# yanqinJiang/Animate3D

Measured on AMD Instinct MI355X. Metric: UNet denoise-steps/sec, 4view×16frame×512² MV-VDM @1/2/4/8 GPU, higher is better.
Workload: dtype bf16; 1 GPU; BASELINE config 2: 4 views x 16 frames x 512^2 px (64x64 latent), CFG-doubled batch V=8 videos, one MVUNetMotionModel.forward per step, SD1.5 MV-VDM UNet 1.53 B params, seeded synthetic weights; parallelism=single GPU

## Files before the change

### animate3d_amd/csrc/gemm_common.h

```cpp
#pragma once
#include "common.h"

struct GemmParams {
  const uint16_t* X; int64_t ldx;
  const uint16_t* W; int64_t ldw;
  const float* bias;
  const uint16_t* rowbias; int64_t rb_div;
  const uint16_t* R; int64_t ldr;
  uint16_t* Y; int64_t ldy;
  int64_t M, N, K;
  float alpha, beta;
  int vec16;
  int out_f32;
  int B, H, Wd, Cin, Ho, Wo, stride, up, He, We;
  int64_t tiles_n, tiles_m;
  int ksplit, nk_item;
  float* ws; int64_t ws_bytes;
  const uint16_t* X2; int64_t ldx2; int64_t K1;
};

constexpr int EPI_LINEAR = 0, EPI_GEGLU = 1;

static inline int a3d_gemm_kernel_of(int flags) { return flags & A3D_GEMM_KERNEL_MASK; }
static inline int a3d_gemm_reserved_cus_of(int flags) { return flags & A3D_GEMM_RESERVED_CUS_MASK; }
// ... 321 lines not shown
      const float4 a1 = *reinterpret_cast<const float4*>(stg + row * SROW + 8 * cc + 4);
      float v[8] = {a0.x, a0.y, a0.z, a0.w, a1.x, a1.y, a1.z, a1.w};
#pragma unroll
      for (int e = 0; e < 8; ++e) v[e] += bv[e];
#pragma unroll
      for (int e = 0; e < 4; ++e) { v[2 * e] += lo16(tb[e]); v[2 * e + 1] += hi16(tb[e]); }
#pragma unroll
      for (int e = 0; e < 8; ++e) v[e] = epi_scale(v[e], p.alpha);
      const u32x4_t tr = rres[pi & 1][j];
#pragma unroll
      for (int e = 0; e < 4; ++e) { v[2 * e] = epi_axpy(v[2 * e], p.beta, lo16(tr[e])); v[2 * e + 1] = epi_axpy(v[2 * e + 1], p.beta, hi16(tr[e])); }
      u32x4_t o;
#pragma unroll
      for (int e = 0; e < 4; ++e) o[e] = pack16(v[2 * e], v[2 * e + 1]);
      *reinterpret_cast<u32x4_t*>(p.Y + m * p.ldy + n) = o;
    }
    wave_lds_fence();
  }
}


__attribute__((visibility("hidden"))) int A3D_FN(a3d_launch_gemm_pp)(int conv, int epi, int nb, hipStream_t stream, const GemmParams& p, int cus);
__attribute__((visibility("hidden"))) int A3D_FN(a3d_launch_gemm_ring)(int nb, hipStream_t stream, const GemmParams& p, int cus);
```

### animate3d_amd/csrc/gemm_conv.hip

```cpp
#include "gemm_common.h"

namespace {

constexpr int BM = 128, BN = 128;
template <int BKT> struct TileCfg {
  static constexpr int LROW = BKT + 8;
  static constexpr int TILE_ELEMS = 128 * LROW;
  static constexpr int STAGE_BYTES = 2 * 2 * TILE_ELEMS * 2;
  static constexpr int EPI_BYTES = 4 * 32 * 68 * 4;
  static constexpr int SMEM_BYTES = STAGE_BYTES > EPI_BYTES ? STAGE_BYTES : EPI_BYTES;
  static constexpr int CPR = BKT / 8;
  static constexpr int RPT = 256 / CPR;
  static constexpr int NPASS = 128 / RPT;
};



template <int CONV, int EPI, int BKT, bool RES>
__global__ __launch_bounds__(256, (BKT == 64 ? 2 : 3)) void gemm_kernel(const GemmParams p) {
  using TC = TileCfg<BKT>;
  constexpr int LROW = TC::LROW, TILE_ELEMS = TC::TILE_ELEMS, NPASS = TC::NPASS, RPT = TC::RPT, BK = BKT;
  extern __shared__ __attribute__((aligned(16))) uint16_t smem[];
  const int tid = threadIdx.x;
  const int lane = tid & 63, wid = tid >> 6;
// ... 491 lines not shown
                                void* Y, int64_t ldy, int64_t M, int64_t N, int64_t K, float alpha, float beta, int flags,
                                void* ws, int64_t ws_bytes, int64_t* ws_needed) {
  return gemm_entry(stream, X, ldx, W, ldw, bias, rowbias, rb_div, R, ldr, Y, ldy, M, N, K, alpha, beta, flags, ws, ws_bytes, ws_needed);
}

extern "C" int A3D_FN(a3d_gemm2)(a3d_stream_t stream, const void* X, int64_t ldx, const void* X2, int64_t ldx2, int64_t K1,
                              const void* W, int64_t ldw, const float* bias, void* Y, int64_t ldy, int64_t M, int64_t N, int64_t K, int flags) {
  GemmParams p = dense_params(X, ldx, W, ldw, bias, nullptr, 1, nullptr, 0, Y, ldy, M, N, K, 1.f, 0.f);
  p.X2 = (const uint16_t*)X2; p.ldx2 = ldx2; p.K1 = K1;
  if (!dense_args_ok(p, 16, 8, 8) || !X2 || K1 <= 0 || K1 >= K || K1 % 64 != 0 || ldx2 % 8 != 0 || !a3d_aligned(16, X2)) return A3D_EINVAL;
  if (!gemm_flags_ok(flags)) return A3D_EINVAL;
  if (ldx2 % 64 != 0 || (uint64_t)ldx2 * 16u >= (1ull << 31)) return A3D_EUNSUPPORTED;
  const int rc = try_launch_persist<0, EPI_LINEAR>((hipStream_t)stream, p, flags);
  return rc == NOT_ELIGIBLE ? A3D_EUNSUPPORTED : rc;
}

extern "C" int A3D_FN(a3d_gemm_f32out)(a3d_stream_t stream, const void* X, int64_t ldx, const void* W, int64_t ldw,
                                    const float* bias, float* Y, int64_t ldy, int64_t M, int64_t N, int64_t K, float alpha) {
  GemmParams p = dense_params(X, ldx, W, ldw, bias, nullptr, 1, nullptr, 0, Y, ldy, M, N, K, alpha, 0.f, true);
  if (!dense_args_ok(p, 16, 8, 4)) return A3D_EINVAL;
  return launch<0>((hipStream_t)stream, p, 0);
}

static int conv_entry(a3d_stream_t stream, const void* X, const void* Wp, const float* bias,
                      const void* rowbias, int64_t rb_div, const void* R, void* Y,
                      int B, int H, int W, int Cin, int Cout, int stride, int up2x, int flags,
                      void* ws, int64_t ws_bytes, int64_t* ws_needed) {
  if (!X || !Wp || !Y || B <= 0 || H <= 0 || W <= 0) return A3D_EINVAL;
  if (Cin % 64 != 0 || Cout % 4 != 0 || (stride != 1 && stride != 2)) return A3D_EINVAL;
  if (up2x < 0 || up2x > 7 || (up2x > 1 && !(up2x & 1)) || (up2x && stride != 1)) return A3D_EINVAL;
  if (!a3d_aligned(16, X, Wp) || !a3d_aligned(16, bias) || !a3d_aligned(8, Y)) return A3D_EINVAL;
  if (rowbias && rb_div <= 0) return A3D_EINVAL;
  const int He = up2x ? 2 * H - ((up2x >> 1) & 1) : H, We = up2x ? 2 * W - ((up2x >> 2) & 1) : W;
  if (He <= 0 || We <= 0) return A3D_EINVAL;
  GemmParams p{};
  p.X = (const uint16_t*)X; p.ldx = Cin; p.W = (const uint16_t*)Wp; p.ldw = (int64_t)9 * Cin;
  p.bias = bias; p.rowbias = (const uint16_t*)rowbias; p.rb_div = rowbias ? rb_div : 1;
  p.R = (const uint16_t*)R; p.ldr = Cout; p.Y = (uint16_t*)Y; p.ldy = Cout;
  p.B = B; p.H = H; p.Wd = W; p.Cin = Cin; p.stride = stride; p.up = up2x ? 1 : 0; p.He = He; p.We = We;
  p.Ho = (He + 2 - 3) / stride + 1; p.Wo = (We + 2 - 3) / stride + 1;
  p.M = (int64_t)B * p.Ho * p.Wo; p.N = Cout; p.K = (int64_t)9 * Cin;
  p.alpha = 1.f; p.beta = 1.f;
  p.vec16 = (Cout % 8 == 0) && a3d_aligned(16, Y, R, rowbias);
  if (ws_needed) { *ws_needed = up2x ? splitk_ws_bytes<2>(p, flags) : splitk_ws_bytes<1>(p, flags); return 0; }
  attach_workspace(p, ws, ws_bytes);
  return up2x ? launch<2>((hipStream_t)stream, p, flags) : launch<1>((hipStream_t)stream, p, flags);
}

extern "C" int A3D_FN(a3d_conv3x3)(a3d_stream_t stream, const void* X, const void* Wp, const float* bias,
                                const void* rowbias, int64_t rb_div, const void* R, void* Y,
                                int B, int H, int W, int Cin, int Cout, int stride, int up2x, int flags) {
  return conv_entry(stream, X, Wp, bias, rowbias, rb_div, R, Y, B, H, W, Cin, Cout, stride, up2x, flags, nullptr, 0, nullptr);
}

extern "C" int A3D_FN(a3d_conv3x3_ws)(a3d_stream_t stream, const void* X, const void* Wp, const float* bias,
                                   const void* rowbias, int64_t rb_div, const void* R, void* Y,
                                   int B, int H, int W, int Cin, int Cout, int stride, int up2x, int flags,
                                   void* ws, int64_t ws_bytes, int64_t* ws_needed) {
  return conv_entry(stream, X, Wp, bias, rowbias, rb_div, R, Y, B, H, W, Cin, Cout, stride, up2x, flags, ws, ws_bytes, ws_needed);
}

extern "C" int A3D_FN(a3d_gemm_geglu)(a3d_stream_t stream, const void* X, int64_t ldx, const void* W, int64_t ldw,
                                   const float* bias, void* Y, int64_t ldy, int64_t M, int64_t N2, int64_t K, int flags) {
  GemmParams p = dense_params(X, ldx, W, ldw, bias, nullptr, 1, nullptr, 0, Y, ldy, M, N2, K, 1.f, 0.f);
  if (!dense_args_ok(p, 16, 64, 8)) return A3D_EINVAL;
  return launch<0, EPI_GEGLU>((hipStream_t)stream, p, flags);
}
```

### animate3d_amd/csrc/temporal_attn.hip

```cpp
#include "common.h"


namespace {

constexpr int SLAB = 320;
constexpr int SL = 40;
constexpr int NSL = SLAB / SL;

struct TAParams {
  const uint16_t* Q; const uint16_t* K; const uint16_t* V; int64_t ld;
  int64_t ldq;
  uint16_t* O; int64_t ldo;
  int videos, frames; int64_t L; int heads; float scale_log2;
  int64_t npix;
  int q_f0, q_frames, kv_fpr; int64_t kv_rs;
};

typedef short s16x4_t __attribute__((ext_vector_type(4)));
typedef _Float16 f16x4_t __attribute__((ext_vector_type(4)));
A3D_DEV f32x4_t mfma16k16(const u32x2_t& a, const u32x2_t& b, const f32x4_t& c) {
#ifdef A3D_STORAGE_F16
  return __builtin_amdgcn_mfma_f32_16x16x16f16(__builtin_bit_cast(f16x4_t, a), __builtin_bit_cast(f16x4_t, b), c, 0, 0, 0);
#else
  return __builtin_amdgcn_mfma_f32_16x16x16bf16_1k(__builtin_bit_cast(s16x4_t, a), __builtin_bit_cast(s16x4_t, b), c, 0, 0, 0);
#endif
}

template <int FP, int D>
__global__ __launch_bounds__(NSL * FP) void temporal_attn_mfma_kernel(const TAParams p) {
  constexpr int ROWB = SLAB + 8;
  constexpr int FB = FP / 16;
  constexpr int KS = (D + 15) / 16;
  constexpr int NH = SLAB / D;
  constexpr int NT = NSL * FP, NW = NT / 64;
  extern __shared__ __attribute__((aligned(16))) uint16_t smem[];
  const int F = p.frames;
  const int tid = threadIdx.x, lane = tid & 63, wid = tid >> 6;
  const int64_t pix = blockIdx.x < p.npix ? (int64_t)blockIdx.x : p.npix - 1;
  const int c0 = blockIdx.y * SLAB;
  const int64_t v = pix / p.L, l = pix % p.L;
  constexpr int chunks = SLAB / 8;

  auto src_of = [&](int it) -> const uint16_t* {
    const int ch = it % chunks;
    const int f = (it / chunks) % F;
    const int ten = it / (chunks * F);
    if (ten == 0) {
      int fq = f - p.q_f0;
      if (fq < 0 || fq >= p.q_frames) fq = 0;
      return p.Q + ((v * p.q_frames + fq) * p.L + l) * p.ldq + c0 + ch * 8;
    }
    const int64_t row = (int64_t)(f / p.kv_fpr) * p.kv_rs + (v * p.kv_fpr + f % p.kv_fpr) * p.L + l;
    return (ten == 1 ? p.K : p.V) + row * p.ld + c0 + ch * 8;
  };
  auto dst_of = [&](int it) -> uint16_t* {
    const int ch = it % chunks;
    const int f = (it / chunks) % F;
    const int ten = it / (chunks * F);
    return smem + ((size_t)ten * F + f) * ROWB + ch * 8;
  };
  const int items = 3 * F * chunks;
  if (F == FP) {
    constexpr int ITEMS = 3 * FP * chunks, NIT = (ITEMS + NT - 1) / NT;
    u32x4_t stg[NIT];
#pragma unroll
    for (int k = 0; k < NIT; ++k) {
      const int it = tid + k * NT;
      if (ITEMS % NT == 0 || it < ITEMS) stg[k] = *reinterpret_cast<const u32x4_t*>(src_of(it));
    }
#pragma unroll
    for (int k = 0; k < NIT; ++k) {
      const int it = tid + k * NT;
      if (ITEMS % NT == 0 || it < ITEMS) *reinterpret_cast<u32x4_t*>(dst_of(it)) = stg[k];
    }
  } else {
    for (int it = tid; it < items; it += NT) *reinterpret_cast<u32x4_t*>(dst_of(it)) = *reinterpret_cast<const u32x4_t*>(src_of(it));
  }
  __syncthreads();

  const int i16 = lane & 15, k4 = lane >> 4;
  uint16_t* const Qs = smem;
  const uint16_t* const Ks = smem + (size_t)F * ROWB;
  const uint16_t* const Vs = smem + (size_t)2 * F * ROWB;
  for (int h = wid; h < NH; h += NW) {
    const int hc = h * D;
    f32x4_t sT[FB][FB];
    u32x2_t qfr[FB][KS];
#pragma unroll
    for (int ib = 0; ib < FB; ++ib) {
      const int fi = 16 * ib + i16 < F ? 16 * ib + i16 : F - 1;
#pragma unroll
      for (int ks = 0; ks < KS; ++ks) {
        u32x2_t w = *reinterpret_cast<const u32x2_t*>(Qs + (size_t)fi * ROWB + hc + 16 * ks + 4 * k4);
        if (16 * ks + 4 * k4 >= D) w = u32x2_t{0u, 0u};
        qfr[ib][ks] = w;
      }
    }
#pragma unroll
    for (int jb = 0; jb < FB; ++jb) {
      const int fj = 16 * jb + i16 < F ? 16 * jb + i16 : F - 1;
      u32x2_t kfr[KS];
#pragma unroll
      for (int ks = 0; ks < KS; ++ks) {
        kfr[ks] = *reinterpret_cast<const u32x2_t*>(Ks + (size_t)fj * ROWB + hc + 16 * ks + 4 * k4);
        if (16 * ks + 4 * k4 >= D) kfr[ks] = u32x2_t{0u, 0u};
      }
#pragma unroll
      for (int ib = 0; ib < FB; ++ib) {
        f32x4_t acc = {0.f, 0.f, 0.f, 0.f};
#pragma unroll
        for (int ks = 0; ks < KS; ++ks) acc = mfma16k16(kfr[ks], qfr[ib][ks], acc);
        sT[jb][ib] = acc;
      }
    }
    u32x2_t pfr[FB][FB];
    float inv[FB];
#pragma unroll
    for (int ib = 0; ib < FB; ++ib) {
      float mx = -INFINITY;
#pragma unroll
      for (int jb = 0; jb < FB; ++jb)
#pragma unroll
        for (int r = 0; r < 4; ++r) {
          const bool ok = 16 * jb + 4 * k4 + r < F;
          sT[jb][ib][r] = ok ? sT[jb][ib][r] * p.scale_log2 : -INFINITY;
          mx = fmaxf(mx, sT[jb][ib][r]);
        }
      mx = fmaxf(mx, __shfl_xor(mx, 16));
      mx = fmaxf(mx, __shfl_xor(mx, 32));
      float sum = 0.f;
#pragma unroll
      for (int jb = 0; jb < FB; ++jb) {
        float e[4];
#pragma unroll
        for (int r = 0; r < 4; ++r) { e[r] = __builtin_amdgcn_exp2f(sT[jb][ib][r] - mx); sum += e[r]; }
        pfr[jb][ib] = u32x2_t{pack16(e[0], e[1]), pack16(e[2], e[3])};
      }
      sum += __shfl_xor(sum, 16);
      sum += __shfl_xor(sum, 32);
      inv[ib] = 1.f / sum;
    }
#pragma unroll
    for (int db = 0; db < KS; ++db) {
      u32x2_t vfr[FB];
#pragma unroll
      for (int jb = 0; jb < FB; ++jb) {
        const int fj = 16 * jb + 4 * k4 + (i16 >> 2) < F ? 16 * jb + 4 * k4 + (i16 >> 2) : F - 1;
        vfr[jb] = lds_tr16_b64(Vs + (size_t)fj * ROWB + hc + 16 * db + 4 * (i16 & 3));
      }
#pragma unroll
      for (int ib = 0; ib < FB; ++ib) {
        f32x4_t o = {0.f, 0.f, 0.f, 0.f};
#pragma unroll
        for (int jb = 0; jb < FB; ++jb) o = mfma16k16(vfr[jb], pfr[jb][ib], o);
        const int fi = 16 * ib + i16;
        if (16 * db + 4 * k4 < D && fi < F) {
          const u32x2_t w = {pack16(o[0] * inv[ib], o[1] * inv[ib]), pack16(o[2] * inv[ib], o[3] * inv[ib])};
          *reinterpret_cast<u32x2_t*>(Qs + (size_t)fi * ROWB + hc + 16 * db + 4 * k4) = w;
        }
      }
    }
  }
  __syncthreads();
  if ((int64_t)blockIdx.x < p.npix) {
    for (int it = tid; it < p.q_frames * chunks; it += NT) {
      const int ch = it % chunks, fq = it / chunks;
      const u32x4_t w = *reinterpret_cast<const u32x4_t*>(Qs + (size_t)(p.q_f0 + fq) * ROWB + ch * 8);
      *reinterpret_cast<u32x4_t*>(p.O + ((v * p.q_frames + fq) * p.L + l) * p.ldo + c0 + ch * 8) = w;
    }
  }
}

template <int FP, int D>
int launch_mfma(hipStream_t s, const TAParams& p, int C) {
  if (p.npix > 0x7fffffffLL) return A3D_EINVAL;
  const size_t lds = (size_t)3 * p.frames * (SLAB + 8) * sizeof(uint16_t);
  static uint64_t attr_done = 0;
  if (int rc = a3d_once_per_device(attr_done, [] {
        return (int)hipFuncSetAttribute(reinterpret_cast<const void*>(&temporal_attn_mfma_kernel<FP, D>),
                                        hipFuncAttributeMaxDynamicSharedMemorySize, 3 * FP * (SLAB + 8) * 2); })) return rc;
  temporal_attn_mfma_kernel<FP, D><<<dim3((unsigned)p.npix, (unsigned)(C / SLAB)), dim3(NSL * FP), lds, s>>>(p);
  return a3d_launch_status();
}

template <int DP>
int launch_dp(hipStream_t s, const TAParams& p, int C) {
  if (p.frames <= 16) return launch_mfma<16, 40 * DP>(s, p, C);
  return launch_mfma<32, 40 * DP>(s, p, C);
}

}

static int temporal_attn_launch(a3d_stream_t stream, const void* Q, int64_t ldq, const void* K, const void* V, int64_t ldqkv, void* O, int64_t ldo,
                                int videos, int frames, int64_t L, int heads, int head_dim, float scale,
                                int q_f0, int q_frames, int kv_fpr, int64_t kv_rs) {
  if (!Q || !K || !V || !O || videos <= 0 || frames <= 0 || frames > 32 || L <= 0 || heads <= 0) return A3D_EINVAL;
  if (q_f0 < 0 || q_frames <= 0 || q_f0 + q_frames > frames || kv_fpr <= 0 || frames % kv_fpr != 0 || kv_rs < 0) return A3D_EINVAL;
  if (ldqkv % 8 || ldo % 8 || ldq % 8) return A3D_EINVAL;
  if ((reinterpret_cast<uintptr_t>(Q) | reinterpret_cast<uintptr_t>(K) | reinterpret_cast<uintptr_t>(V) |
       reinterpret_cast<uintptr_t>(O)) & 15u) return A3D_EINVAL;
  const int C = heads * head_dim;
  if (C % SLAB != 0) return A3D_EUNSUPPORTED;
  TAParams p{};
  p.Q = (const uint16_t*)Q; p.K = (const uint16_t*)K; p.V = (const uint16_t*)V; p.ld = ldqkv; p.ldq = ldq;
  p.O = (uint16_t*)O; p.ldo = ldo; p.videos = videos; p.frames = frames; p.L = L; p.heads = heads;
  p.scale_log2 = scale * 1.4426950408889634f;
  p.npix = (int64_t)videos * L;
  p.q_f0 = q_f0; p.q_frames = q_frames; p.kv_fpr = kv_fpr; p.kv_rs = kv_rs;
  hipStream_t s = (hipStream_t)stream;
  switch (head_dim) {
    case 40: return launch_dp<1>(s, p, C);
    case 80: return launch_dp<2>(s, p, C);
    case 160: return launch_dp<4>(s, p, C);
    default: return A3D_EUNSUPPORTED;
// ... 17 lines not shown
```

### animate3d_amd/hip_ops.py

```python
from __future__ import annotations

import ctypes
import os
from dataclasses import dataclass
from typing import Optional

import torch

_LIB_PATH = os.path.join(os.path.dirname(os.path.abspath(__file__)), "lib", "libanimate3d_hip.so")
_lib = None

c_i64, c_int, c_f32, c_f64, c_vp = ctypes.c_int64, ctypes.c_int, ctypes.c_float, ctypes.c_double, ctypes.c_void_p


class _RowMapC(ctypes.Structure):
    _fields_ = [("gdiv", c_i64), ("ga", c_i64), ("gb", c_i64), ("seg_len", c_i64), ("seg_stride", c_i64), ("ld", c_i64)]


class StageAdamEntry(ctypes.Structure):
    _fields_ = [("p", c_vp), ("g", c_vp), ("m", c_vp), ("v", c_vp), ("step", c_vp), ("n", c_i64), ("lr", c_f64)]


STAGE_ADAM_MAX_TENSORS = 32
STAGE_ADAM_BEGIN, STAGE_ADAM_CHECK, STAGE_ADAM_UPDATE = 1, 2, 4
# ... 14 lines not shown
def rowmap_rows(m: RowMap, groups: int, step: int, length: int, device="cpu") -> torch.Tensor:
    g = torch.arange(0, groups, step, device=device).view(-1, 1)
    s = torch.arange(length, device=device).view(1, -1)
    return ((g // m.gdiv) * m.ga + (g % m.gdiv) * m.gb + (s // m.seg_len) * m.seg_stride + s % m.seg_len).reshape(-1)


def rowmap_covers(m: RowMap, groups: int, step: int, length: int, rows: int, device="cpu") -> bool:
    if (groups + step - 1) // step * length != rows:
        return False
    idx = rowmap_rows(m, groups, step, length, device)
    return bool(int(idx.min()) >= 0 and int(idx.max()) < rows and torch.unique(idx).numel() == rows)


_SIGNATURES = {
    "a3d_version": (ctypes.c_char_p, []),
    "a3d_gemm_bf16": (c_int, [c_vp, c_vp, c_i64, c_vp, c_i64, c_vp, c_vp, c_i64, c_vp, c_i64, c_vp, c_i64, c_i64, c_i64, c_i64, c_f32, c_f32, c_int]),
    "a3d_gemm_ws_bf16": (c_int, [c_vp, c_vp, c_i64, c_vp, c_i64, c_vp, c_vp, c_i64, c_vp, c_i64, c_vp, c_i64, c_i64, c_i64, c_i64, c_f32, c_f32, c_int,
                                 c_vp, c_i64, ctypes.POINTER(c_i64)]),
    "a3d_gemm2_bf16": (c_int, [c_vp, c_vp, c_i64, c_vp, c_i64, c_i64, c_vp, c_i64, c_vp, c_vp, c_i64, c_i64, c_i64, c_i64, c_int]),
    "a3d_gemm_geglu_bf16": (c_int, [c_vp, c_vp, c_i64, c_vp, c_i64, c_vp, c_vp, c_i64, c_i64, c_i64, c_i64, c_int]),
    "a3d_conv3x3_bf16": (c_int, [c_vp, c_vp, c_vp, c_vp, c_vp, c_i64, c_vp, c_vp, c_int, c_int, c_int, c_int, c_int, c_int, c_int, c_int]),
    "a3d_conv3x3_ws_bf16": (c_int, [c_vp, c_vp, c_vp, c_vp, c_vp, c_i64, c_vp, c_vp, c_int, c_int, c_int, c_int, c_int, c_int, c_int, c_int,
                                    c_vp, c_i64, ctypes.POINTER(c_i64)]),
    "a3d_flash_attn_bf16": (c_int, [c_vp, c_vp, c_vp, c_vp, c_vp, ctypes.POINTER(_RowMapC), ctypes.POINTER(_RowMapC), ctypes.POINTER(_RowMapC),
                                    c_int, c_int, c_int, c_i64, c_i64, c_f32, c_f32, c_int]),
    "a3d_flash_attn_counted_bf16": (c_int, [c_vp, c_vp, c_vp, c_vp, c_vp, ctypes.POINTER(_RowMapC), ctypes.POINTER(_RowMapC), ctypes.POINTER(_RowMapC),
                                            c_int, c_int, c_int, c_i64, c_i64, c_f32, c_f32, c_int, c_vp]),
    "a3d_flash_attn2_bf16": (c_int, [c_vp, c_vp, c_vp, c_vp, c_vp, c_vp, c_vp, ctypes.POINTER(_RowMapC), ctypes.POINTER(_RowMapC), ctypes.POINTER(_RowMapC),
                                     ctypes.POINTER(_RowMapC), c_int, c_int, c_int, c_i64, c_i64, c_i64, c_f32, c_f32, c_f32, c_int]),
    "a3d_temporal_attn_bf16": (c_int, [c_vp, c_vp, c_vp, c_vp, c_i64, c_vp, c_i64, c_int, c_int, c_i64, c_int, c_int, c_f32]),
    "a3d_temporal_attn_sharded_bf16": (c_int, [c_vp, c_vp, c_i64, c_vp, c_vp, c_i64, c_vp, c_i64, c_int, c_int, c_i64, c_int, c_int, c_f32,
                                               c_int, c_int, c_int, c_i64]),
    "a3d_group_norm_ws_floats": (c_i64, [c_int, c_i64, c_int]),
    "a3d_group_norm_plan": (c_int, [c_i64, c_int, c_int, ctypes.POINTER(c_int)]),
    "a3d_group_norm_bf16": (c_int, [c_vp, c_vp, c_vp, c_vp, c_vp, c_vp, c_int, c_i64, c_int, c_int, c_f32, c_int]),
    "a3d_group_norm2_bf16": (c_int, [c_vp, c_vp, c_int, c_vp, c_int, c_vp, c_vp, c_vp, c_vp, c_int, c_i64, c_int, c_f32, c_int]),
    "a3d_group_norm_sums_bf16": (c_int, [c_vp, c_vp, c_vp, c_vp, c_int, c_i64, c_int, c_int]),
    "a3d_group_norm_apply_bf16": (c_int, [c_vp, c_vp, c_vp, c_vp, c_vp, c_vp, c_int, c_i64, c_int, c_int, c_int]),
    "a3d_layer_norm_bf16": (c_int, [c_vp, c_vp, c_vp, c_vp, c_vp, c_vp, c_i64, c_int, c_f32, c_vp, c_i64, c_i64, c_vp, c_i64, c_i64]),
    "a3d_geglu_bf16": (c_int, [c_vp, c_vp, c_i64, c_vp, c_i64, c_i64, c_i64]),
    "a3d_silu_bf16": (c_int, [c_vp, c_vp, c_vp, c_i64]),
    "a3d_activation_bf16": (c_int, [c_vp, c_vp, c_vp, c_i64, c_int]),
    "a3d_concat_bf16": (c_int, [c_vp, c_vp, c_i64, c_vp, c_i64, c_vp, c_i64]),
    "a3d_timestep_embed_bf16": (c_int, [c_vp, c_vp, c_vp, c_int, c_int]),
    "a3d_im2col_in": (c_int, [c_vp, c_vp, c_int, c_vp, c_int, c_int, c_int, c_int, c_int]),
    "a3d_unpack_out": (c_int, [c_vp, c_vp, c_vp, c_int, c_int, c_int, c_int, c_int, c_int]),
    "a3d_gemm_f32out_bf16": (c_int, [c_vp, c_vp, c_i64, c_vp, c_i64, c_vp, c_vp, c_i64, c_i64, c_i64, c_i64, c_f32]),
    "a3d_softmax_rows_f32_bf16": (c_int, [c_vp, c_vp, c_i64, c_vp, c_i64, c_i64, c_i64]),
    "a3d_softmax_rows_bwd_bf16": (c_int, [c_vp, c_vp, c_i64, c_vp, c_i64, c_vp, c_i64, c_i64, c_i64, c_f32]),
    "a3d_im2col_in_bwd": (c_int, [c_vp, c_vp, c_vp, c_int, c_int, c_int, c_int, c_int, c_f32]),
    "a3d_channel_mix_f32": (c_int, [c_vp, c_vp, c_vp, c_vp, c_vp, c_int, c_int, c_int, c_i64, c_f32]),
    "a3d_cfg_ddim_step_f32": (c_int, [c_vp, c_vp, c_vp, c_vp, c_vp, c_i64, c_int, c_int, c_i64, c_f32, c_f32, c_f32]),
    "a3d_flash_attn_bwd_bf16": (c_int, [c_vp, c_vp, c_vp, c_vp, c_vp, c_vp, c_vp, c_vp, c_vp, c_vp,
                                        ctypes.POINTER(_RowMapC), ctypes.POINTER(_RowMapC), ctypes.POINTER(_RowMapC), ctypes.POINTER(_RowMapC),
                                        ctypes.POINTER(_RowMapC), c_int, c_int, c_int, c_i64, c_i64, c_int, c_f32, c_f32, c_int]),
# ... 77 lines not shown
    if _lib is None:
        if not os.path.exists(_LIB_PATH):
            raise RuntimeError(f"{_LIB_PATH} is missing: run `python -m animate3d_amd.build` (or __graft_entry__.build()). "
                               "There is no CPU fallback for the MI355X kernels.")
        lib = ctypes.CDLL(_LIB_PATH)
        for name, (res, args) in _SIGNATURES.items():
            fn = getattr(lib, name)
            fn.restype, fn.argtypes = res, args
        _lib = lib
    return _lib


GN_PLAN_FIELDS = ("fused", "sg", "nx", "ny", "threads", "rmax", "stream")


def group_norm_plan(rows: int, C: int, groups: int) -> dict:
    out = (c_int * len(GN_PLAN_FIELDS))()
    _check(load_library().a3d_group_norm_plan(rows, C, groups, out), f"a3d_group_norm_plan rows={rows} C={C} groups={groups}")
    plan = dict(zip(GN_PLAN_FIELDS, out))
    plan["iters"] = -(-rows // plan["ny"]) if plan["fused"] else 0
    return plan


def _check(rc: int, what: str):
    if rc != 0:
        kind = {-1: "A3D_EINVAL (shape/alignment precondition)", -2: "A3D_EUNSUPPORTED"}.get(rc, f"hipError {rc}")
        raise RuntimeError(f"{what} failed: {kind}")


def _p(t: Optional[torch.Tensor]):
    return None if t is None else t.data_ptr()


def on_model_device(method):
    import functools

    @functools.wraps(method)
    def wrapper(self, *args, **kwargs):
        dev = self.device
        if dev.type == "cuda" and torch.cuda.current_device() != (dev.index if dev.index is not None else torch.cuda.current_device()):
            with torch.cuda.device(dev):
                return method(self, *args, **kwargs)
        return method(self, *args, **kwargs)
    return wrapper


# ... 577 lines not shown
```

### include/animate3d_hip.h

```cpp
#ifndef ANIMATE3D_HIP_H
#define ANIMATE3D_HIP_H

#include <stdint.h>

#ifdef __cplusplus
extern "C" {
#endif

typedef void* a3d_stream_t;

enum {
  A3D_OK = 0,
  A3D_EINVAL = -1,
  A3D_EUNSUPPORTED = -2
};

enum { A3D_F32 = 0, A3D_BF16 = 1, A3D_F16 = 2 };

const char* a3d_version(void);

typedef struct a3d_rowmap {
  int64_t gdiv, ga, gb;
  int64_t seg_len, seg_stride;
  int64_t ld;
// ... 4 lines not shown
#define A3D_GEMM_TILE128 0x100
#define A3D_GEMM_RING 0x200
int a3d_gemm_bf16(a3d_stream_t stream, const void* X, int64_t ldx, const void* W, int64_t ldw,
                  const float* bias, const void* rowbias, int64_t rb_div, const void* R, int64_t ldr,
                  void* Y, int64_t ldy, int64_t M, int64_t N, int64_t K, float alpha, float beta, int flags);

int a3d_gemm_ws_bf16(a3d_stream_t stream, const void* X, int64_t ldx, const void* W, int64_t ldw,
                     const float* bias, const void* rowbias, int64_t rb_div, const void* R, int64_t ldr,
                     void* Y, int64_t ldy, int64_t M, int64_t N, int64_t K, float alpha, float beta, int flags,
                     void* ws, int64_t ws_bytes, int64_t* ws_needed);

int a3d_gemm2_bf16(a3d_stream_t stream, const void* X, int64_t ldx, const void* X2, int64_t ldx2, int64_t K1,
                   const void* W, int64_t ldw, const float* bias, void* Y, int64_t ldy, int64_t M, int64_t N, int64_t K, int flags);

int a3d_gemm_f32out_bf16(a3d_stream_t stream, const void* X, int64_t ldx, const void* W, int64_t ldw,
                         const float* bias, float* Y, int64_t ldy, int64_t M, int64_t N, int64_t K, float alpha);

int a3d_gemm_geglu_bf16(a3d_stream_t stream, const void* X, int64_t ldx, const void* W, int64_t ldw,
                        const float* bias, void* Y, int64_t ldy, int64_t M, int64_t N2, int64_t K, int flags);

int a3d_conv3x3_bf16(a3d_stream_t stream, const void* X, const void* Wp, const float* bias,
                     const void* rowbias, int64_t rb_div, const void* R, void* Y,
                     int B, int H, int W, int Cin, int Cout, int stride, int up2x, int flags);

int a3d_conv3x3_ws_bf16(a3d_stream_t stream, const void* X, const void* Wp, const float* bias,
                        const void* rowbias, int64_t rb_div, const void* R, void* Y,
                        int B, int H, int W, int Cin, int Cout, int stride, int up2x, int flags,
                        void* ws, int64_t ws_bytes, int64_t* ws_needed);

#define A3D_ATTN_ACCUMULATE 1
#define A3D_ATTN_CAUSAL 2
#define A3D_ATTN_EXACT 4
#define A3D_ATTN_PLAIN 8
int a3d_flash_attn_bf16(a3d_stream_t stream, const void* Q, const void* K, const void* V, void* O,
                        const a3d_rowmap* qmap, const a3d_rowmap* kmap, const a3d_rowmap* omap,
                        int groups, int heads, int head_dim, int64_t q_len, int64_t kv_len,
                        float scale, float out_scale, int accumulate);

int a3d_flash_attn_counted_bf16(a3d_stream_t stream, const void* Q, const void* K, const void* V, void* O,
                                const a3d_rowmap* qmap, const a3d_rowmap* kmap, const a3d_rowmap* omap,
                                int groups, int heads, int head_dim, int64_t q_len, int64_t kv_len,
                                float scale, float out_scale, int accumulate, unsigned int* counters);

int a3d_flash_attn2_bf16(a3d_stream_t stream, const void* Q, const void* K, const void* V, const void* K2, const void* V2, void* O,
                         const a3d_rowmap* qmap, const a3d_rowmap* kmap, const a3d_rowmap* kmap2, const a3d_rowmap* omap,
                         int groups, int heads, int head_dim, int64_t q_len, int64_t kv_len, int64_t kv_len2,
                         float scale, float out_scale, float out_scale2, int accumulate);

int a3d_temporal_attn_bf16(a3d_stream_t stream, const void* Q, const void* K, const void* V, int64_t ldqkv,
                           void* O, int64_t ldo, int videos, int frames, int64_t L, int heads,
                           int head_dim, float scale);

int a3d_temporal_attn_sharded_bf16(a3d_stream_t stream, const void* Q, int64_t ldq, const void* K, const void* V, int64_t ldkv,
                                   void* O, int64_t ldo, int videos, int frames, int64_t L, int heads,
                                   int head_dim, float scale, int q_f0, int q_frames, int kv_frames_per_block,
                                   int64_t kv_block_stride);

int64_t a3d_group_norm_ws_floats(int B, int64_t rows, int groups);
int a3d_group_norm_bf16(a3d_stream_t stream, const void* X, void* Y, const float* gamma, const float* beta,
                        float* ws, int B, int64_t rows, int C, int groups, float eps, int silu);

int a3d_group_norm_plan(int64_t rows, int C, int groups, int* out);

int a3d_group_norm2_bf16(a3d_stream_t stream, const void* Xa, int Ca, const void* Xb, int Cb, void* Y, const float* gamma,
                         const float* beta, float* ws, int B, int64_t rows, int groups, float eps, int silu);

int a3d_group_norm_sums_bf16(a3d_stream_t stream, const void* X, float* ws, double* sums, int B, int64_t rows, int C, int groups);
int a3d_group_norm_apply_bf16(a3d_stream_t stream, const void* X, void* Y, const float* gamma, const float* beta,
                              const float* stats, int B, int64_t rows, int C, int groups, int silu);

int a3d_layer_norm_bf16(a3d_stream_t stream, const void* X, void* Y1, void* Y2, const float* gamma,
                        const float* beta, int64_t M, int C, float eps,
                        const void* pe1, int64_t pe1_div, int64_t pe1_mod,
                        const void* pe2, int64_t pe2_div, int64_t pe2_mod);
// ... 295 lines not shown
```

Before: 2.451 denoise-steps/s.

## Add small-Cout direct conv3x3 kernel and multi-pixel walking temporal attention

```diff
diff --git a/animate3d_amd/csrc/conv_small.hip b/animate3d_amd/csrc/conv_small.hip
--- /dev/null
+++ b/animate3d_amd/csrc/conv_small.hip
@@ -0,0 +1,149 @@
+#include "gemm_common.h"
+
+namespace {
+
+constexpr int CS_TH = 4, CS_TW = 64;
+constexpr int CS_WR = CS_TH + 2, CS_WC = CS_TW + 2;
+constexpr int CS_PIX = 64 + 8;
+constexpr int CS_WIN_ELEMS = CS_WR * CS_WC * CS_PIX;
+constexpr int CS_CHUNKS = CS_WR * CS_WC * 8;
+constexpr int CS_NT = 64 * CS_TH;
+constexpr int CS_NLD = (CS_CHUNKS + CS_NT - 1) / CS_NT;
+constexpr int CS_WPAD = 8;
+constexpr size_t CS_LDS_MAX = 160 * 1024;
+
+__global__ __launch_bounds__(CS_NT) void conv3x3_small_kernel(const GemmParams p, const int tiles_x, const int tiles_y) {
+  extern __shared__ __attribute__((aligned(16))) uint16_t smem[];
+  uint16_t* const win = smem;
+  uint16_t* const wl = smem + CS_WIN_ELEMS;
+  const int tid = threadIdx.x, lane = tid & 63;
+  const int wid = __builtin_amdgcn_readfirstlane(tid >> 6);
+  const int l31 = lane & 31, g = lane >> 5;
+  const int Cin = p.Cin, Cout = (int)p.N, K = 9 * Cin, wrow = K + CS_WPAD;
+
+  const uint32_t lid = xcd_remap32(blockIdx.x, gridDim.x);
+  const int tx = (int)(lid % (uint32_t)tiles_x);
+  const int ty = (int)((lid / (uint32_t)tiles_x) % (uint32_t)tiles_y);
+  const int b = (int)(lid / ((uint32_t)tiles_x * (uint32_t)tiles_y));
+  const int y0 = ty * CS_TH, x0 = tx * CS_TW;
+  const uint16_t* const Xb = p.X + (int64_t)b * p.H * p.Wd * Cin;
+
+  int off[CS_NLD];
+  uint32_t okmask = 0;
+#pragma unroll
+  for (int k = 0; k < CS_NLD; ++k) {
+    const int it = tid + k * CS_NT;
+    const int ch = it & 7, pc = it >> 3;
+    const int row = pc / CS_WC, col = pc - row * CS_WC;
+    const int y = y0 - 1 + row, x = x0 - 1 + col;
+    const bool ok = it < CS_CHUNKS && y >= 0 && y < p.H && x >= 0 && x < p.Wd;
+    off[k] = ok ? (y * p.Wd + x) * Cin + ch * 8 : 0;
+    okmask |= ok ? 1u << k : 0u;
+  }
+  u32x4_t stg[CS_NLD];
+  auto load_win = [&](int c64) {
+#pragma unroll
+    for (int k = 0; k < CS_NLD; ++k) stg[k] = *reinterpret_cast<const u32x4_t*>(Xb + off[k] + c64 * 64);
+  };
+  auto store_win = [&]() {
+#pragma unroll
+    for (int k = 0; k < CS_NLD; ++k) {
+      const int it = tid + k * CS_NT;
+      if (CS_CHUNKS % CS_NT != 0 && it >= CS_CHUNKS) continue;
+      const u32x4_t v = (okmask >> k) & 1u ? stg[k] : u32x4_t{0u, 0u, 0u, 0u};
+      *reinterpret_cast<u32x4_t*>(win + (it >> 3) * CS_PIX + (it & 7) * 8) = v;
+    }
+  };
+
+  load_win(0);
+  {
+    const int cpr = K / 8;
+    for (int it = tid; it < Cout * cpr; it += CS_NT) {
+      const int n = it / cpr, c = it - n * cpr;
+      *reinterpret_cast<u32x4_t*>(wl + n * wrow + c * 8) = *reinterpret_cast<const u32x4_t*>(p.W + (int64_t)n * p.ldw + c * 8);
+    }
+  }
+  store_win();
+  __syncthreads();
+
+  f32x16_t acc[2];
+#pragma unroll
+  for (int j = 0; j < 2; ++j)
+#pragma unroll
+    for (int r = 0; r < 16; ++r) acc[j][r] = 0.f;
+
+  const bool row_live = y0 + wid < p.H;
+  const uint16_t* const wfr = wl + (l31 < Cout ? l31 : Cout - 1) * wrow + g * 8;
+  const uint16_t* const afr = win + (wid * CS_WC + l31) * CS_PIX + g * 8;
+  const int nslice = Cin / 64;
+  for (int c64 = 0; c64 < nslice; ++c64) {
+    if (c64 + 1 < nslice) load_win(c64 + 1);
+    if (row_live) {
+#pragma unroll
+      for (int t = 0; t < 9; ++t) {
+        const int ky = t / 3, kx = t % 3;
+        const uint16_t* const wt = wfr + t * Cin + c64 * 64;
+        const uint16_t* const at = afr + (ky * CS_WC + kx) * CS_PIX;
+#pragma unroll
+        for (int ks = 0; ks < 4; ++ks) {
+          const u32x4_t fw = *reinterpret_cast<const u32x4_t*>(wt + ks * 16);
+#pragma unroll
+          for (int j = 0; j < 2; ++j) {
+            const u32x4_t fa = *reinterpret_cast<const u32x4_t*>(at + j * 32 * CS_PIX + ks * 16);
+            acc[j] = mfma32(fw, fa, acc[j]);
+          }
+        }
+      }
+    }
+    if (c64 + 1 < nslice) {
+      __syncthreads();
+      store_win();
+      __syncthreads();
+    }
+  }
+
+  const int y = y0 + wid;
+  if (row_live && 4 * g < Cout) {
+    float bv[4];
+#pragma unroll
+    for (int e = 0; e < 4; ++e) bv[e] = p.bias ? p.bias[4 * g + e] : 0.f;
+#pragma unroll
+    for (int j = 0; j < 2; ++j) {
+      const int x = x0 + 32 * j + l31;
+      if (x >= p.Wd) continue;
+      float v[4];
+#pragma unroll
+      for (int e = 0; e < 4; ++e) v[e] = epi_scale(acc[j][e] + bv[e], p.alpha);
+      u32x2_t o;
+      o[0] = pack16(v[0], v[1]);
+      o[1] = pack16(v[2], v[3]);
+      const int64_t m = ((int64_t)b * p.H + y) * p.Wd + x;
+      *reinterpret_cast<u32x2_t*>(p.Y + m * p.ldy + 4 * g) = o;
+    }
+  }
+}
+
+}
+
+bool A3D_FN(a3d_conv3x3_small_ok)(const GemmParams& p) {
+  if (p.N <= 0 || p.N > 8 || p.N % 4 != 0 || p.stride != 1 || p.up || p.rowbias || p.R || p.Cin <= 0 || p.Cin % 64 != 0) return false;
+  if (p.B <= 0 || p.H <= 0 || p.Wd <= 0) return false;
+  const size_t lds = ((size_t)CS_WIN_ELEMS + (size_t)p.N * (9 * (size_t)p.Cin + CS_WPAD)) * sizeof(uint16_t);
+  if (lds > CS_LDS_MAX) return false;
+  if ((int64_t)p.H * p.Wd * p.Cin >= (1ll << 31)) return false;
+  const int64_t nblk = (int64_t)p.B * ((p.Wd + CS_TW - 1) / CS_TW) * ((p.H + CS_TH - 1) / CS_TH);
+  return nblk <= 0x7fffffffLL;
+}
+
+int A3D_FN(a3d_launch_conv3x3_small)(hipStream_t s, const GemmParams& p) {
+  if (!A3D_FN(a3d_conv3x3_small_ok)(p)) return A3D_EUNSUPPORTED;
+  const size_t lds = ((size_t)CS_WIN_ELEMS + (size_t)p.N * (9 * (size_t)p.Cin + CS_WPAD)) * sizeof(uint16_t);
+  const int tiles_x = (p.Wd + CS_TW - 1) / CS_TW, tiles_y = (p.H + CS_TH - 1) / CS_TH;
+  const int64_t nblk = (int64_t)p.B * tiles_x * tiles_y;
+  static uint64_t attr_done = 0;
+  if (int rc = a3d_once_per_device(attr_done, [] {
+        return (int)hipFuncSetAttribute(reinterpret_cast<const void*>(&conv3x3_small_kernel), hipFuncAttributeMaxDynamicSharedMemorySize,
+                                        (int)CS_LDS_MAX); })) return rc;
+  conv3x3_small_kernel<<<dim3((unsigned)nblk), dim3(CS_NT), lds, s>>>(p, tiles_x, tiles_y);
+  return a3d_launch_status();
+}
diff --git a/animate3d_amd/csrc/gemm_common.h b/animate3d_amd/csrc/gemm_common.h
--- a/animate3d_amd/csrc/gemm_common.h
+++ b/animate3d_amd/csrc/gemm_common.h
@@ -367,3 +367,5 @@
 
 __attribute__((visibility("hidden"))) int A3D_FN(a3d_launch_gemm_pp)(int conv, int epi, int nb, hipStream_t stream, const GemmParams& p, int cus);
 __attribute__((visibility("hidden"))) int A3D_FN(a3d_launch_gemm_ring)(int nb, hipStream_t stream, const GemmParams& p, int cus);
+__attribute__((visibility("hidden"))) bool A3D_FN(a3d_conv3x3_small_ok)(const GemmParams& p);
+__attribute__((visibility("hidden"))) int A3D_FN(a3d_launch_conv3x3_small)(hipStream_t stream, const GemmParams& p);
diff --git a/animate3d_amd/csrc/gemm_conv.hip b/animate3d_amd/csrc/gemm_conv.hip
--- a/animate3d_amd/csrc/gemm_conv.hip
+++ b/animate3d_amd/csrc/gemm_conv.hip
@@ -537,6 +537,22 @@
   return launch<0>((hipStream_t)stream, p, 0);
 }
 
+static bool conv_takes_small(const GemmParams& p, int flags) {
+  return gemm_flags_ok(flags) && a3d_gemm_kernel_of(flags) == 0 && A3D_FN(a3d_conv3x3_small_ok)(p);
+}
+
+#ifndef A3D_STORAGE_F16
+extern "C" int a3d_conv3x3_plan(int B, int H, int W, int Cin, int Cout, int stride, int up2x, int has_rowbias, int has_residual, int flags) {
+  if (B <= 0 || H <= 0 || W <= 0 || Cin <= 0 || Cin % 64 != 0 || Cout <= 0 || Cout % 4 != 0 || (stride != 1 && stride != 2)) return A3D_EINVAL;
+  if (!gemm_flags_ok(flags)) return A3D_EINVAL;
+  GemmParams p{};
+  p.B = B; p.H = H; p.Wd = W; p.Cin = Cin; p.N = Cout; p.stride = stride; p.up = up2x ? 1 : 0;
+  p.rowbias = has_rowbias ? reinterpret_cast<const uint16_t*>(&p) : nullptr;
+  p.R = has_residual ? reinterpret_cast<const uint16_t*>(&p) : nullptr;
+  return conv_takes_small(p, flags) ? 1 : 0;
+}
+#endif
+
 static int conv_entry(a3d_stream_t stream, const void* X, const void* Wp, const float* bias,
                       const void* rowbias, int64_t rb_div, const void* R, void* Y,
                       int B, int H, int W, int Cin, int Cout, int stride, int up2x, int flags,
@@ -559,6 +575,7 @@
   p.vec16 = (Cout % 8 == 0) && a3d_aligned(16, Y, R, rowbias);
   if (ws_needed) { *ws_needed = up2x ? splitk_ws_bytes<2>(p, flags) : splitk_ws_bytes<1>(p, flags); return 0; }
   attach_workspace(p, ws, ws_bytes);
+  if (conv_takes_small(p, flags)) return A3D_FN(a3d_launch_conv3x3_small)((hipStream_t)stream, p);
   return up2x ? launch<2>((hipStream_t)stream, p, flags) : launch<1>((hipStream_t)stream, p, flags);
 }
 
diff --git a/animate3d_amd/csrc/temporal_attn.hip b/animate3d_amd/csrc/temporal_attn.hip
--- a/animate3d_amd/csrc/temporal_attn.hip
+++ b/animate3d_amd/csrc/temporal_attn.hip
@@ -1,5 +1,6 @@
+#include <stdlib.h>
+
 #include "common.h"
-
 
 namespace {
 
@@ -27,12 +28,102 @@
 }
 
 template <int FP, int D>
-__global__ __launch_bounds__(NSL * FP) void temporal_attn_mfma_kernel(const TAParams p) {
+A3D_DEV void ta_attend_slab(uint16_t* const smem, const int F, const float scale_log2, const int lane, const int wid) {
+#pragma clang fp contract(off)
   constexpr int ROWB = SLAB + 8;
   constexpr int FB = FP / 16;
   constexpr int KS = (D + 15) / 16;
   constexpr int NH = SLAB / D;
-  constexpr int NT = NSL * FP, NW = NT / 64;
+  constexpr int NW = NSL * FP / 64;
+  const int i16 = lane & 15, k4 = lane >> 4;
+  uint16_t* const Qs = smem;
+  const uint16_t* const Ks = smem + (size_t)F * ROWB;
+  const uint16_t* const Vs = smem + (size_t)2 * F * ROWB;
+  for (int h = wid; h < NH; h += NW) {
+    const int hc = h * D;
+    f32x4_t sT[FB][FB];
+    u32x2_t qfr[FB][KS];
+#pragma unroll
+    for (int ib = 0; ib < FB; ++ib) {
+      const int fi = 16 * ib + i16 < F ? 16 * ib + i16 : F - 1;
+#pragma unroll
+      for (int ks = 0; ks < KS; ++ks) {
+        u32x2_t w = *reinterpret_cast<const u32x2_t*>(Qs + (size_t)fi * ROWB + hc + 16 * ks + 4 * k4);
+        if (16 * ks + 4 * k4 >= D) w = u32x2_t{0u, 0u};
+        qfr[ib][ks] = w;
+      }
+    }
+#pragma unroll
+    for (int jb = 0; jb < FB; ++jb) {
+      const int fj = 16 * jb + i16 < F ? 16 * jb + i16 : F - 1;
+      u32x2_t kfr[KS];
+#pragma unroll
+      for (int ks = 0; ks < KS; ++ks) {
+        kfr[ks] = *reinterpret_cast<const u32x2_t*>(Ks + (size_t)fj * ROWB + hc + 16 * ks + 4 * k4);
+        if (16 * ks + 4 * k4 >= D) kfr[ks] = u32x2_t{0u, 0u};
+      }
+#pragma unroll
+      for (int ib = 0; ib < FB; ++ib) {
+        f32x4_t acc = {0.f, 0.f, 0.f, 0.f};
+#pragma unroll
+        for (int ks = 0; ks < KS; ++ks) acc = mfma16k16(kfr[ks], qfr[ib][ks], acc);
+        sT[jb][ib] = acc;
+      }
+    }
+    u32x2_t pfr[FB][FB];
+    float inv[FB];
+#pragma unroll
+    for (int ib = 0; ib < FB; ++ib) {
+      float mx = -INFINITY;
+#pragma unroll
+      for (int jb = 0; jb < FB; ++jb)
+#pragma unroll
+        for (int r = 0; r < 4; ++r) {
+          const bool ok = 16 * jb + 4 * k4 + r < F;
+          sT[jb][ib][r] = ok ? sT[jb][ib][r] * scale_log2 : -INFINITY;
+          mx = fmaxf(mx, sT[jb][ib][r]);
+        }
+      mx = fmaxf(mx, __shfl_xor(mx, 16));
+      mx = fmaxf(mx, __shfl_xor(mx, 32));
+      float sum = 0.f;
+#pragma unroll
+      for (int jb = 0; jb < FB; ++jb) {
+        float e[4];
+#pragma unroll
+        for (int r = 0; r < 4; ++r) { e[r] = __builtin_amdgcn_exp2f(sT[jb][ib][r] - mx); sum += e[r]; }
+        pfr[jb][ib] = u32x2_t{pack16(e[0], e[1]), pack16(e[2], e[3])};
+      }
+      sum += __shfl_xor(sum, 16);
+      sum += __shfl_xor(sum, 32);
+      inv[ib] = 1.f / sum;
+    }
+#pragma unroll
+    for (int db = 0; db < KS; ++db) {
+      u32x2_t vfr[FB];
+#pragma unroll
+      for (int jb = 0; jb < FB; ++jb) {
+        const int fj = 16 * jb + 4 * k4 + (i16 >> 2) < F ? 16 * jb + 4 * k4 + (i16 >> 2) : F - 1;
+        vfr[jb] = lds_tr16_b64(Vs + (size_t)fj * ROWB + hc + 16 * db + 4 * (i16 & 3));
+      }
+#pragma unroll
+      for (int ib = 0; ib < FB; ++ib) {
+        f32x4_t o = {0.f, 0.f, 0.f, 0.f};
+#pragma unroll
+        for (int jb = 0; jb < FB; ++jb) o = mfma16k16(vfr[jb], pfr[jb][ib], o);
+        const int fi = 16 * ib + i16;
+        if (16 * db + 4 * k4 < D && fi < F) {
+          const u32x2_t w = {pack16(o[0] * inv[ib], o[1] * inv[ib]), pack16(o[2] * inv[ib], o[3] * inv[ib])};
+          *reinterpret_cast<u32x2_t*>(Qs + (size_t)fi * ROWB + hc + 16 * db + 4 * k4) = w;
+        }
+      }
+    }
+  }
+}
+
+template <int FP, int D>
+__global__ __launch_bounds__(NSL * FP) void temporal_attn_mfma_kernel(const TAParams p) {
+  constexpr int ROWB = SLAB + 8;
+  constexpr int NT = NSL * FP;
   extern __shared__ __attribute__((aligned(16))) uint16_t smem[];
   const int F = p.frames;
   const int tid = threadIdx.x, lane = tid & 63, wid = tid >> 6;
@@ -78,103 +169,112 @@
   }
   __syncthreads();
 
-  const int i16 = lane & 15, k4 = lane >> 4;
-  uint16_t* const Qs = smem;
-  const uint16_t* const Ks = smem + (size_t)F * ROWB;
-  const uint16_t* const Vs = smem + (size_t)2 * F * ROWB;
-  for (int h = wid; h < NH; h += NW) {
-    const int hc = h * D;
-    f32x4_t sT[FB][FB];
-    u32x2_t qfr[FB][KS];
-#pragma unroll
-    for (int ib = 0; ib < FB; ++ib) {
-      const int fi = 16 * ib + i16 < F ? 16 * ib + i16 : F - 1;
-#pragma unroll
-      for (int ks = 0; ks < KS; ++ks) {
-        u32x2_t w = *reinterpret_cast<const u32x2_t*>(Qs + (size_t)fi * ROWB + hc + 16 * ks + 4 * k4);
-        if (16 * ks + 4 * k4 >= D) w = u32x2_t{0u, 0u};
-        qfr[ib][ks] = w;
-      }
-    }
-#pragma unroll
-    for (int jb = 0; jb < FB; ++jb) {
-      const int fj = 16 * jb + i16 < F ? 16 * jb + i16 : F - 1;
-      u32x2_t kfr[KS];
-#pragma unroll
-      for (int ks = 0; ks < KS; ++ks) {
-        kfr[ks] = *reinterpret_cast<const u32x2_t*>(Ks + (size_t)fj * ROWB + hc + 16 * ks + 4 * k4);
-        if (16 * ks + 4 * k4 >= D) kfr[ks] = u32x2_t{0u, 0u};
-      }
-#pragma unroll
-      for (int ib = 0; ib < FB; ++ib) {
-        f32x4_t acc = {0.f, 0.f, 0.f, 0.f};
-#pragma unroll
-        for (int ks = 0; ks < KS; ++ks) acc = mfma16k16(kfr[ks], qfr[ib][ks], acc);
-        sT[jb][ib] = acc;
-      }
-    }
-    u32x2_t pfr[FB][FB];
-    float inv[FB];
-#pragma unroll
-    for (int ib = 0; ib < FB; ++ib) {
-      float mx = -INFINITY;
-#pragma unroll
-      for (int jb = 0; jb < FB; ++jb)
-#pragma unroll
-        for (int r = 0; r < 4; ++r) {
-          const bool ok = 16 * jb + 4 * k4 + r < F;
-          sT[jb][ib][r] = ok ? sT[jb][ib][r] * p.scale_log2 : -INFINITY;
-          mx = fmaxf(mx, sT[jb][ib][r]);
-        }
-      mx = fmaxf(mx, __shfl_xor(mx, 16));
-      mx = fmaxf(mx, __shfl_xor(mx, 32));
-      float sum = 0.f;
-#pragma unroll
-      for (int jb = 0; jb < FB; ++jb) {
-        float e[4];
-#pragma unroll
-        for (int r = 0; r < 4; ++r) { e[r] = __builtin_amdgcn_exp2f(sT[jb][ib][r] - mx); sum += e[r]; }
-        pfr[jb][ib] = u32x2_t{pack16(e[0], e[1]), pack16(e[2], e[3])};
-      }
-      sum += __shfl_xor(sum, 16);
-      sum += __shfl_xor(sum, 32);
-      inv[ib] = 1.f / sum;
-    }
-#pragma unroll
-    for (int db = 0; db < KS; ++db) {
-      u32x2_t vfr[FB];
-#pragma unroll
-      for (int jb = 0; jb < FB; ++jb) {
-        const int fj = 16 * jb + 4 * k4 + (i16 >> 2) < F ? 16 * jb + 4 * k4 + (i16 >> 2) : F - 1;
-        vfr[jb] = lds_tr16_b64(Vs + (size_t)fj * ROWB + hc + 16 * db + 4 * (i16 & 3));
-      }
-#pragma unroll
-      for (int ib = 0; ib < FB; ++ib) {
-        f32x4_t o = {0.f, 0.f, 0.f, 0.f};
-#pragma unroll
-        for (int jb = 0; jb < FB; ++jb) o = mfma16k16(vfr[jb], pfr[jb][ib], o);
-        const int fi = 16 * ib + i16;
-        if (16 * db + 4 * k4 < D && fi < F) {
-          const u32x2_t w = {pack16(o[0] * inv[ib], o[1] * inv[ib]), pack16(o[2] * inv[ib], o[3] * inv[ib])};
-          *reinterpret_cast<u32x2_t*>(Qs + (size_t)fi * ROWB + hc + 16 * db + 4 * k4) = w;
-        }
-      }
-    }
-  }
+  ta_attend_slab<FP, D>(smem, F, p.scale_log2, lane, wid);
   __syncthreads();
   if ((int64_t)blockIdx.x < p.npix) {
     for (int it = tid; it < p.q_frames * chunks; it += NT) {
       const int ch = it % chunks, fq = it / chunks;
-      const u32x4_t w = *reinterpret_cast<const u32x4_t*>(Qs + (size_t)(p.q_f0 + fq) * ROWB + ch * 8);
+      const u32x4_t w = *reinterpret_cast<const u32x4_t*>(smem + (size_t)(p.q_f0 + fq) * ROWB + ch * 8);
       *reinterpret_cast<u32x4_t*>(p.O + ((v * p.q_frames + fq) * p.L + l) * p.ldo + c0 + ch * 8) = w;
     }
   }
+}
+
+template <int FP, int D>
+__global__ __launch_bounds__(NSL * FP, (FP == 16 ? 3 : 2)) void temporal_attn_walk_kernel(const TAParams p, const int walk) {
+  constexpr int ROWB = SLAB + 8;
+  constexpr int NT = NSL * FP;
+  constexpr int chunks = SLAB / 8;
+  constexpr int NG = NT / chunks;
+  static_assert(NG % 3 == 0 && (NG / 3) * 16 == FP, "a staging group = one tensor x 16 frames");
+  extern __shared__ __attribute__((aligned(16))) uint16_t smem[];
+  const int tid = threadIdx.x, lane = tid & 63, wid = tid >> 6;
+  const int c0 = blockIdx.y * SLAB;
+  const int64_t pix0 = (int64_t)blockIdx.x * walk;
+  const int64_t pix1 = pix0 + walk < p.npix ? pix0 + walk : p.npix;
+
+  const int sg = tid / chunks, ch = tid - sg * chunks;
+  const bool stager = sg < NG;
+  const int ten = sg % 3, fb = (sg / 3) * 16;
+  const uint16_t* const tbase = (ten == 0 ? p.Q : (ten == 1 ? p.K : p.V)) + c0 + ch * 8;
+  const int64_t tld = ten == 0 ? p.ldq : p.ld;
+  const int tfpv = ten == 0 ? p.q_frames : p.kv_fpr;
+  int foff[16];
+#pragma unroll
+  for (int k = 0; k < 16; ++k) {
+    const int f = fb + k;
+    int64_t row;
+    if (ten == 0) {
+      int fq = f - p.q_f0;
+      if (fq < 0 || fq >= p.q_frames) fq = 0;
+      row = (int64_t)fq * p.L;
+    } else {
+      row = (int64_t)(f / p.kv_fpr) * p.kv_rs + (int64_t)(f % p.kv_fpr) * p.L;
+    }
+    foff[k] = (int)(row * tld);
+  }
+  uint16_t* const sdst = smem + ((size_t)ten * FP + fb) * ROWB + ch * 8;
+  u32x4_t stg[16];
+  auto load_pixel = [&](int64_t pix) {
+    const int64_t v = pix / p.L, l = pix % p.L;
+    const uint16_t* const src = tbase + (v * tfpv * p.L + l) * tld;
+    if (stager) {
+#pragma unroll
+      for (int k = 0; k < 16; ++k) stg[k] = *reinterpret_cast<const u32x4_t*>(src + foff[k]);
+    }
+  };
+  load_pixel(pix0);
+  for (int64_t pix = pix0; pix < pix1; ++pix) {
+    if (stager) {
+#pragma unroll
+      for (int k = 0; k < 16; ++k) *reinterpret_cast<u32x4_t*>(sdst + k * ROWB) = stg[k];
+    }
+    __syncthreads();
+    if (pix + 1 < pix1) load_pixel(pix + 1);
+    ta_attend_slab<FP, D>(smem, FP, p.scale_log2, lane, wid);
+    __syncthreads();
+    const int64_t v = pix / p.L, l = pix % p.L;
+    for (int it = tid; it < p.q_frames * chunks; it += NT) {
+      const int ch = it % chunks, fq = it / chunks;
+      const u32x4_t w = *reinterpret_cast<const u32x4_t*>(smem + (size_t)(p.q_f0 + fq) * ROWB + ch * 8);
+      *reinterpret_cast<u32x4_t*>(p.O + ((v * p.q_frames + fq) * p.L + l) * p.ldo + c0 + ch * 8) = w;
+    }
+    if (pix + 1 < pix1) __syncthreads();
+  }
+}
+
+constexpr int TA_WALK_MAX = 64;
+constexpr int64_t TA_ROUND = 5 * 256;
+inline int ta_walk_of(int frames, int64_t npix, int slabs) {
+  if (frames != 16 && frames != 32) return 1;
+  if (const char* e = getenv("A3D_TEMPORAL_WALK")) {
+    const long n = strtol(e, nullptr, 10);
+    return n <= 1 ? 1 : (n > TA_WALK_MAX ? TA_WALK_MAX : (int)n);
+  }
+  const int64_t total = npix * slabs;
+  if (frames != 16 || total <= TA_ROUND) return 1;
+  for (int w : {2, 4, 8})
+    if (total <= w * TA_ROUND) return w;
+  return 2;
 }
 
 template <int FP, int D>
 int launch_mfma(hipStream_t s, const TAParams& p, int C) {
   if (p.npix > 0x7fffffffLL) return A3D_EINVAL;
   const size_t lds = (size_t)3 * p.frames * (SLAB + 8) * sizeof(uint16_t);
+  int walk = ta_walk_of(p.frames, p.npix, C / SLAB);
+  const int64_t span_q = (int64_t)(p.q_frames - 1) * p.L * p.ldq;
+  const int64_t span_kv = ((int64_t)(p.frames / p.kv_fpr - 1) * p.kv_rs + (int64_t)(p.kv_fpr - 1) * p.L) * p.ld;
+  if (span_q >= (1ll << 31) || span_kv >= (1ll << 31)) walk = 1;
+  if (walk > 1) {
+    static uint64_t attr_done_walk = 0;
+    if (int rc = a3d_once_per_device(attr_done_walk, [] {
+          return (int)hipFuncSetAttribute(reinterpret_cast<const void*>(&temporal_attn_walk_kernel<FP, D>),
+                                          hipFuncAttributeMaxDynamicSharedMemorySize, 3 * FP * (SLAB + 8) * 2); })) return rc;
+    const int64_t nwg = (p.npix + walk - 1) / walk;
+    temporal_attn_walk_kernel<FP, D><<<dim3((unsigned)nwg, (unsigned)(C / SLAB)), dim3(NSL * FP), lds, s>>>(p, walk);
+    return a3d_launch_status();
+  }
   static uint64_t attr_done = 0;
   if (int rc = a3d_once_per_device(attr_done, [] {
         return (int)hipFuncSetAttribute(reinterpret_cast<const void*>(&temporal_attn_mfma_kernel<FP, D>),
@@ -190,6 +290,16 @@
 }
 
 }
+
+#ifndef A3D_STORAGE_F16
+extern "C" int a3d_temporal_attn_plan(int videos, int frames, int64_t L, int heads, int head_dim) {
+  if (videos <= 0 || frames <= 0 || frames > 32 || L <= 0 || heads <= 0) return A3D_EINVAL;
+  if (head_dim != 40 && head_dim != 80 && head_dim != 160) return A3D_EUNSUPPORTED;
+  const int C = heads * head_dim;
+  if (C % SLAB != 0) return A3D_EUNSUPPORTED;
+  return ta_walk_of(frames, (int64_t)videos * L, C / SLAB);
+}
+#endif
 
 static int temporal_attn_launch(a3d_stream_t stream, const void* Q, int64_t ldq, const void* K, const void* V, int64_t ldqkv, void* O, int64_t ldo,
                                 int videos, int frames, int64_t L, int heads, int head_dim, float scale,
diff --git a/animate3d_amd/hip_ops.py b/animate3d_amd/hip_ops.py
--- a/animate3d_amd/hip_ops.py
+++ b/animate3d_amd/hip_ops.py
@@ -60,6 +60,7 @@
     "a3d_conv3x3_bf16": (c_int, [c_vp, c_vp, c_vp, c_vp, c_vp, c_i64, c_vp, c_vp, c_int, c_int, c_int, c_int, c_int, c_int, c_int, c_int]),
     "a3d_conv3x3_ws_bf16": (c_int, [c_vp, c_vp, c_vp, c_vp, c_vp, c_i64, c_vp, c_vp, c_int, c_int, c_int, c_int, c_int, c_int, c_int, c_int,
                                     c_vp, c_i64, ctypes.POINTER(c_i64)]),
+    "a3d_conv3x3_plan": (c_int, [c_int, c_int, c_int, c_int, c_int, c_int, c_int, c_int, c_int, c_int]),
     "a3d_flash_attn_bf16": (c_int, [c_vp, c_vp, c_vp, c_vp, c_vp, ctypes.POINTER(_RowMapC), ctypes.POINTER(_RowMapC), ctypes.POINTER(_RowMapC),
                                     c_int, c_int, c_int, c_i64, c_i64, c_f32, c_f32, c_int]),
     "a3d_flash_attn_counted_bf16": (c_int, [c_vp, c_vp, c_vp, c_vp, c_vp, ctypes.POINTER(_RowMapC), ctypes.POINTER(_RowMapC), ctypes.POINTER(_RowMapC),
@@ -69,6 +70,7 @@
     "a3d_temporal_attn_bf16": (c_int, [c_vp, c_vp, c_vp, c_vp, c_i64, c_vp, c_i64, c_int, c_int, c_i64, c_int, c_int, c_f32]),
     "a3d_temporal_attn_sharded_bf16": (c_int, [c_vp, c_vp, c_i64, c_vp, c_vp, c_i64, c_vp, c_i64, c_int, c_int, c_i64, c_int, c_int, c_f32,
                                                c_int, c_int, c_int, c_i64]),
+    "a3d_temporal_attn_plan": (c_int, [c_int, c_int, c_i64, c_int, c_int]),
     "a3d_group_norm_ws_floats": (c_i64, [c_int, c_i64, c_int]),
     "a3d_group_norm_plan": (c_int, [c_i64, c_int, c_int, ctypes.POINTER(c_int)]),
     "a3d_group_norm_bf16": (c_int, [c_vp, c_vp, c_vp, c_vp, c_vp, c_vp, c_int, c_i64, c_int, c_int, c_f32, c_int]),
@@ -192,6 +194,21 @@
     return plan
 
 
+def conv3x3_takes_small_kernel(B: int, H: int, W: int, Cin: int, Cout: int, *, stride: int = 1, up2x: bool = False, rowbias: bool = False,
+                               residual: bool = False, tile128: bool = False) -> bool:
+    rc = load_library().a3d_conv3x3_plan(B, H, W, Cin, Cout, stride, 1 if up2x else 0, int(rowbias), int(residual), 0x100 if tile128 else 0)
+    if rc < 0:
+        _check(rc, f"a3d_conv3x3_plan B={B} H={H} W={W} Cin={Cin} Cout={Cout} stride={stride}")
+    return rc == 1
+
+
+def temporal_attn_walk(videos: int, frames: int, L: int, heads: int, head_dim: int) -> int:
+    rc = load_library().a3d_temporal_attn_plan(videos, frames, L, heads, head_dim)
+    if rc < 0:
+        _check(rc, f"a3d_temporal_attn_plan videos={videos} frames={frames} L={L} heads={heads} head_dim={head_dim}")
+    return rc
+
+
 def _check(rc: int, what: str):
     if rc != 0:
         kind = {-1: "A3D_EINVAL (shape/alignment precondition)", -2: "A3D_EUNSUPPORTED"}.get(rc, f"hipError {rc}")
diff --git a/include/animate3d_hip.h b/include/animate3d_hip.h
--- a/include/animate3d_hip.h
+++ b/include/animate3d_hip.h
@@ -50,6 +50,8 @@
 int a3d_conv3x3_bf16(a3d_stream_t stream, const void* X, const void* Wp, const float* bias,
                      const void* rowbias, int64_t rb_div, const void* R, void* Y,
                      int B, int H, int W, int Cin, int Cout, int stride, int up2x, int flags);
+
+int a3d_conv3x3_plan(int B, int H, int W, int Cin, int Cout, int stride, int up2x, int has_rowbias, int has_residual, int flags);
 
 int a3d_conv3x3_ws_bf16(a3d_stream_t stream, const void* X, const void* Wp, const float* bias,
                         const void* rowbias, int64_t rb_div, const void* R, void* Y,
@@ -78,6 +80,8 @@
 int a3d_temporal_attn_bf16(a3d_stream_t stream, const void* Q, const void* K, const void* V, int64_t ldqkv,
                            void* O, int64_t ldo, int videos, int frames, int64_t L, int heads,
                            int head_dim, float scale);
+
+int a3d_temporal_attn_plan(int videos, int frames, int64_t L, int heads, int head_dim);
 
 int a3d_temporal_attn_sharded_bf16(a3d_stream_t stream, const void* Q, int64_t ldq, const void* K, const void* V, int64_t ldkv,
                                    void* O, int64_t ldo, int videos, int frames, int64_t L, int heads,
```

New measurement: 2.457 denoise-steps/s, median of 4. Within noise of the previous version (+0.2%).
